# pacificclimate/VIC

Measured on AMD Instinct MI355X. Metric: cell-timesteps/s, higher is better.
Workload: dtype f64

## Files before the change

vic_amd/build.py:

```python
import os
import subprocess
import sys

HERE = os.path.dirname(os.path.abspath(__file__))
ROOT = os.path.dirname(HERE)
SRC = os.path.join(HERE, "csrc", "vicgpu_api.hip")
OUT = os.path.join(HERE, "libvicgpu.so")
HIPCC = os.environ.get("HIPCC", "/opt/rocm/bin/hipcc")
FLAGS = ["--offload-arch=gfx950", "-O3", "-ffp-contract=off", "-std=c++17", "-fPIC", "-shared", "-ftrivial-auto-var-init=zero",
         "-mllvm", "-sgpr-regalloc=basic",
         "-I" + os.path.join(ROOT, "include"), "-I" + os.path.join(HERE, "csrc")]


def needs_build():
    if not os.path.exists(OUT):
        return True
    t = os.path.getmtime(OUT)
    deps = [os.path.join(HERE, "csrc", f) for f in os.listdir(os.path.join(HERE, "csrc"))] + [os.path.join(ROOT, "include", f) for f in os.listdir(os.path.join(ROOT, "include"))]
    return any(os.path.getmtime(d) > t for d in deps)


RESOURCE_LIMITS = {
    "vic_hru_step<3, false>": (256, 3200),
    "vic_hru_step<3, true>": (256, 1800),
    "vic_hru_step<10, true>": (256, 2200),
    "vic_fd_stage<10, true, false>": (256, 800),
    "vic_fd_stage<10, false, false>": (256, 600),
    "vic_hru_step<50, true>": (256, 5200),
    "vic_fd_stage<50, true, false>": (256, 4500),
    "vic_fd_stage<50, true, true>": (256, 4500),
    "vic_fd_stage<50, false, false>": (256, 5300),
    "vic_fd_stage<50, false, true>": (256, 6300),
    "vic_surf_eval": (256, 0),
    "vic::vic_profile_solve_reg<10": (256, 128),
    "vic::vic_profile_solve_lockstep": (256, 0),
    "vic::vic_put_": (256, 0),
    "vic_cell_reduce": (128, 0),
}


def parse_resources(remarks):
    import re
    kern, cur = {}, None
    for line in remarks.splitlines():
        m = re.search(r"remark: .*?Function Name: (\S+)", line)
        if m:
            cur = m.group(1); kern[cur] = {}; continue
        m = re.search(r"remark: .*?\s{2,}([A-Za-z ]+?)(?: \[[^\]]*\])?: (\S+) \[-Rpass", line)
        if m and cur:
            kern[cur][m.group(1).strip()] = m.group(2)
    return kern


def resource_table(kern):
    import re
    names = list(kern)
    dem = subprocess.run(["c++filt"] + names, stdout=subprocess.PIPE, text=True).stdout.splitlines() if names else []
    rows = []
    for name, dm in zip(names, dem):
        v = kern[name]
        short = re.sub(r"\(.*", "", dm).replace("void ", "")
        rows.append((short, v.get("VGPRs", "?"), v.get("AGPRs", "?"), v.get("TotalSGPRs", "?"), v.get("ScratchSize", "?"),
                     v.get("VGPRs Spill", "?"), v.get("SGPRs Spill", "?"), v.get("Occupancy", "?")))
    rows.sort()
    return rows


def check_resources(rows):
    bad = []
    for r in rows:
        for prefix, (max_vgpr, max_scratch) in RESOURCE_LIMITS.items():
            if r[0].startswith(prefix):
                try:
                    if int(r[1]) > max_vgpr or int(r[4]) > max_scratch:
                        bad.append("%s: %s VGPRs, %s B scratch (limit %d / %d)" % (r[0], r[1], r[4], max_vgpr, max_scratch))
                except ValueError:
                    pass
    return bad


def build(force=False, extra=(), verbose=False, out=OUT):
    if not force and out == OUT and not needs_build():
        return OUT
    cmd = [HIPCC] + FLAGS + list(extra) + ["-Rpass-analysis=kernel-resource-usage", SRC, "-o", out]
    if verbose:
        print(" ".join(cmd))
    p = subprocess.run(cmd, stdout=subprocess.PIPE, stderr=subprocess.STDOUT, text=True)
    if p.returncode != 0:
        sys.stderr.write(p.stdout)
        raise subprocess.CalledProcessError(p.returncode, cmd)
    rows = resource_table(parse_resources(p.stdout))
    with open(os.path.splitext(out)[0] + ".resources.txt", "w") as f:
        f.write("%-62s %5s %5s %5s %8s %6s %6s %5s\n" % ("kernel", "VGPR", "AGPR", "SGPR", "scratchB", "vspill", "sspill", "occ"))
        for r in rows:
            f.write("%-62s %5s %5s %5s %8s %6s %6s %5s\n" % ((r[0][:62],) + r[1:]))
    bad = check_resources(rows)
    if bad and not extra:
        raise RuntimeError("kernel resource limits exceeded (vic_amd/build.py RESOURCE_LIMITS):\n  " + "\n  ".join(bad))
    return OUT


if __name__ == "__main__":
    args = [a for a in sys.argv[1:] if a != "-f"]
    out = OUT
    if "-o" in args:
        i = args.index("-o")
        out = os.path.abspath(args[i + 1])
        del args[i:i + 2]
    build(force="-f" in sys.argv, extra=args, verbose=True, out=out)
```

vic_amd/csrc/vicgpu_api.hip:

```cpp
#include <hip/hip_runtime.h>
#include <stdio.h>
#include <stdlib.h>
#include <string.h>
#include <algorithm>
#include <atomic>
#include <chrono>
#include <string>
#include <thread>
#include <vector>
#include "vicgpu.h"
#include <cstddef>
#include <type_traits>
#include "vic_glacier.hpp"
#include "vic_profile.hpp"
#include "vic_putdata.hpp"

using namespace vic;

#define HIPIGN(call) do { hipError_t ign_ = (call); (void)ign_; } while (0)
#define HIPCHK(ctx, call)                                                                              \
  do {                                                                                                 \
    hipError_t e_ = (call);                                                                            \
    if (e_ != hipSuccess) {                                                                            \
      (ctx)->err = std::string(#call) + ": " + hipGetErrorString(e_);                                  \
// ... 179 lines not shown
template <int NN>
VIC_DEV void load_state(const KArgs& a, int g, HruWork<NN>& w, bool node_props = true) {
  const int Nn = a.o.Nnode;
  const size_t nh = a.nhru;
  const double* __restrict__ sd = a.sd;
  const int* __restrict__ si = a.si;
#define SD(row) sd[(size_t)(row) * nh + g]
#define SI(row) si[(size_t)(row) * nh + g]
#pragma unroll
  for (int l = 0; l < 3; l++) { w.moist[l] = SD(SD_MOIST0 + l); w.ice[l] = SD(SD_ICE0 + l); w.layer_T[l] = SD(SD_LAYER_T0 + l); w.evap[l] = 0; }
  SoilEnergy& so = w.so; SnowEnergy& se = w.se; Snow& s = w.snow;
  so.snow_flux = SD(SD_SNOW_FLUX); so.grnd_flux = SD(SD_GRND_FLUX); so.deltaH = SD(SD_DELTAH); so.fusion = SD(SD_FUSION);
  so.LongUnderOut = SD(SD_LONGUNDEROUT); se.Tfoliage = SD(SD_TFOLIAGE);
  s.albedo = SD(SD_SNOW_ALBEDO); s.coldcontent = SD(SD_SNOW_COLDCONTENT); s.coverage = SD(SD_SNOW_COVERAGE);
  s.density = SD(SD_SNOW_DENSITY); s.depth = SD(SD_SNOW_DEPTH); s.pack_temp = SD(SD_SNOW_PACK_TEMP);
  s.pack_water = SD(SD_SNOW_PACK_WATER); s.snow_canopy = SD(SD_SNOW_CANOPY); s.surf_temp = SD(SD_SNOW_SURF_TEMP);
  s.surf_water = SD(SD_SNOW_SURF_WATER); s.swq = SD(SD_SNOW_SWQ); s.tmp_int_storage = SD(SD_SNOW_TMP_INT_STORAGE);
  s.store_swq = SD(SD_SNOW_STORE_SWQ); s.store_coverage = SD(SD_SNOW_STORE_COVERAGE); s.swq_slope = SD(SD_SNOW_SWQ_SLOPE);
  s.max_swq = SD(SD_SNOW_MAX_SWQ);
  s.blowing_flux = 0; s.canopy_vapor_flux = 0; s.mass_error = 0; s.melt = 0; s.Qnet = 0; s.surface_flux = 0; s.vapor_flux = 0;
  w.vv.Wdew = SD(SD_WDEW); w.vv.canopyevap = 0; w.vv.throughfall = 0;
  w.Tcanopy = SD(SD_TCANOPY); so.Tsurf = SD(SD_TSURF); se.AlbedoOver = SD(SD_ALBEDO_OVER); so.AlbedoUnder = SD(SD_ALBEDO_UNDER);
  se.canopy_advection = SD(SD_CANOPY_ADVECTION); se.canopy_latent = SD(SD_CANOPY_LATENT);
  se.canopy_latent_sub = SD(SD_CANOPY_LATENT_SUB); se.canopy_sensible = SD(SD_CANOPY_SENSIBLE);
  se.canopy_refreeze = SD(SD_CANOPY_REFREEZE);
  se.advected_sensible = so.advected_sensible = SD(SD_ADVECTED_SENSIBLE);
  se.advection = so.advection = SD(SD_ADVECTION);
  se.deltaCC = so.deltaCC = SD(SD_DELTACC);
  se.refreeze_energy = so.refreeze_energy = SD(SD_REFREEZE_ENERGY);
  so.melt_energy = SD(SD_MELT_ENERGY);
  se.error = so.error = SD(SD_ERROR);
  se.latent = so.latent = SD(SD_LATENT); se.latent_sub = so.latent_sub = SD(SD_LATENT_SUB);
  se.sensible = so.sensible = SD(SD_SENSIBLE);
  se.snow_flux = so.snow_flux;
  se.LongOverIn = SD(SD_LONGOVERIN); se.NetLongOver = SD(SD_NETLONGOVER); se.NetShortOver = SD(SD_NETSHORTOVER);
  se.ShortOverIn = SD(SD_SHORTOVERIN);
  so.NetShortGrnd = 0; so.NetLongUnder = SD(SD_NETLONGUNDER); so.NetShortUnder = 0;
  w.gl.surf_temp = SD(SD_GLAC_SURF_TEMP); w.gl.water_storage = SD(SD_GLAC_WATER_STORAGE);
  w.gl.cum_mass_balance = SD(SD_GLAC_CUM_MASS_BALANCE);
  w.gl.cold_content = NAN; w.gl.Qnet = NAN; w.gl.mass_balance = NAN; w.gl.ice_mass_balance = 0; w.gl.accumulation = NAN;
  w.gl.melt = NAN; w.gl.vapor_flux = NAN; w.gl.outflow = NAN; w.gl.outflow_coef = NAN; w.gl.inflow = NAN;
  w.deltaCC_glac = 0; w.glacier_flux = 0; w.glacier_melt_energy = 0;
  so.kappa[0] = so.kappa[1] = so.Cs[0] = so.Cs[1] = 0;
#pragma unroll
  for (int f = 0; f < 3; f++) { so.fdepth[f] = 0; so.tdepth[f] = 0; }
#pragma unroll
  for (int n = 0; n < NN; n++) {
    if (n < Nn) {
      w.nd.T[n] = SD(VICGPU_SD_NODE(SDN_T, n, Nn));
      if (node_props) {
        w.nd.moist[n] = SD(VICGPU_SD_NODE(SDN_MOIST, n, Nn)); w.nd.ice[n] = SD(VICGPU_SD_NODE(SDN_ICE, n, Nn));
        w.nd.kappa[n] = SD(VICGPU_SD_NODE(SDN_KAPPA, n, Nn)); w.nd.Cs[n] = SD(VICGPU_SD_NODE(SDN_CS, n, Nn));
      } else { w.nd.moist[n] = 0; w.nd.ice[n] = 0; w.nd.kappa[n] = 0; w.nd.Cs[n] = 0; }
      w.nd.fbflag[n] = SI(VICGPU_SI_NODE(SIN_T_FBFLAG, n, Nn)); w.nd.fbcount[n] = SI(VICGPU_SI_NODE(SIN_T_FBCOUNT, n, Nn));
    } else {
      w.nd.T[n] = 0; w.nd.moist[n] = 0; w.nd.ice[n] = 0; w.nd.kappa[n] = 0; w.nd.Cs[n] = 0; w.nd.fbflag[n] = 0; w.nd.fbcount[n] = 0;
    }
  }
  s.last_snow = SI(SI_SNOW_LAST_SNOW); s.MELTING = SI(SI_SNOW_MELTING); s.snow = SI(SI_SNOW_SNOW); s.store_snow = SI(SI_SNOW_STORE_SNOW);
  s.surf_temp_fbcount = SI(SI_SNOW_SURF_TEMP_FBCOUNT); s.surf_temp_fbflag = SI(SI_SNOW_SURF_TEMP_FBFLAG);
  so.Tsurf_fbcount = SI(SI_TSURF_FBCOUNT); so.Tsurf_fbflag = SI(SI_TSURF_FBFLAG);
  se.Tfoliage_fbcount = SI(SI_TFOLIAGE_FBCOUNT); se.Tfoliage_fbflag = SI(SI_TFOLIAGE_FBFLAG);
  so.frozen = SI(SI_FROZEN); so.Nfrost = SI(SI_NFROST); so.Nthaw = SI(SI_NTHAW);
  w.gl.surf_temp_fbcount = SI(SI_GLAC_SURF_TEMP_FBCOUNT); w.gl.surf_temp_fbflag = SI(SI_GLAC_SURF_TEMP_FBFLAG);
#undef SD
#undef SI
}

template <int NN>
VIC_DEV void load_node_props(const KArgs& a, int g, Nodes<NN>& nd) {
  const int Nn = a.o.Nnode;
  const size_t nh = a.nhru;
  const double* __restrict__ sd = a.sd;
#pragma unroll
  for (int n = 0; n < NN; n++) {
    if (n < Nn) {
      nd.moist[n] = sd[(size_t)VICGPU_SD_NODE(SDN_MOIST, n, Nn) * nh + g]; nd.ice[n] = sd[(size_t)VICGPU_SD_NODE(SDN_ICE, n, Nn) * nh + g];
      nd.kappa[n] = sd[(size_t)VICGPU_SD_NODE(SDN_KAPPA, n, Nn) * nh + g]; nd.Cs[n] = sd[(size_t)VICGPU_SD_NODE(SDN_CS, n, Nn) * nh + g];
    }
  }
}

template <int NN>
VIC_DEV void load_untouched_state(const KArgs& a, int g, HruWork<NN>& w) {
  const int Nn = a.o.Nnode;
  const size_t nh = a.nhru;
  const double* __restrict__ sd = a.sd;
  const int* __restrict__ si = a.si;
#pragma unroll
  for (int l = 0; l < 3; l++) {
    w.moist[l] = sd[(size_t)(SD_MOIST0 + l) * nh + g]; w.ice[l] = sd[(size_t)(SD_ICE0 + l) * nh + g];
    w.layer_T[l] = sd[(size_t)(SD_LAYER_T0 + l) * nh + g]; w.evap[l] = 0;
  }
  w.vv.Wdew = sd[(size_t)SD_WDEW * nh + g]; w.vv.canopyevap = 0; w.vv.throughfall = 0;
  SoilEnergy& so = w.so;
  so.deltaCC = 0; so.refreeze_energy = 0; so.deltaH = 0; so.fusion = 0; so.grnd_flux = 0; so.latent = 0; so.latent_sub = 0; so.sensible = 0;
  so.snow_flux = 0; so.error = 0; so.NetShortGrnd = 0; so.NetLongUnder = 0; so.NetShortUnder = 0; so.LongUnderOut = 0; so.AlbedoUnder = 0;
  so.melt_energy = 0; so.Tsurf = 0; so.kappa[0] = so.kappa[1] = so.Cs[0] = so.Cs[1] = 0;
#pragma unroll
  for (int f = 0; f < 3; f++) { so.fdepth[f] = 0; so.tdepth[f] = 0; }
  so.advected_sensible = sd[(size_t)SD_ADVECTED_SENSIBLE * nh + g];
  so.Tsurf_fbflag = 0; so.Tsurf_fbcount = si[(size_t)SI_TSURF_FBCOUNT * nh + g];
  so.frozen = 0; so.Nfrost = 0; so.Nthaw = si[(size_t)SI_NTHAW * nh + g];
  w.Tcanopy = 0;
  w.gl.surf_temp = sd[(size_t)SD_GLAC_SURF_TEMP * nh + g]; w.gl.water_storage = sd[(size_t)SD_GLAC_WATER_STORAGE * nh + g];
  w.gl.cum_mass_balance = sd[(size_t)SD_GLAC_CUM_MASS_BALANCE * nh + g];
  w.gl.cold_content = NAN; w.gl.Qnet = NAN; w.gl.mass_balance = NAN; w.gl.ice_mass_balance = 0; w.gl.accumulation = NAN;
  w.gl.melt = NAN; w.gl.vapor_flux = NAN; w.gl.outflow = NAN; w.gl.outflow_coef = NAN; w.gl.inflow = NAN;
  w.gl.surf_temp_fbcount = si[(size_t)SI_GLAC_SURF_TEMP_FBCOUNT * nh + g]; w.gl.surf_temp_fbflag = si[(size_t)SI_GLAC_SURF_TEMP_FBFLAG * nh + g];
  w.deltaCC_glac = 0; w.glacier_flux = 0; w.glacier_melt_energy = 0;
#pragma unroll
  for (int n = 0; n < NN; n++) {
    w.nd.T[n] = 0; w.nd.moist[n] = 0; w.nd.ice[n] = 0; w.nd.kappa[n] = 0; w.nd.Cs[n] = 0; w.nd.fbflag[n] = 0;
    w.nd.fbcount[n] = (n < Nn) ? si[(size_t)VICGPU_SI_NODE(SIN_T_FBCOUNT, n, Nn) * nh + g] : 0;
  }
#pragma unroll
  for (int p = 0; p < NPET; p++) w.pot_evap[p] = 0;
}

template <int NN>
VIC_DEV void store_state(const KArgs& a, int g, const HruWork<NN>& w) {
  const int Nn = a.o.Nnode;
  const size_t nh = a.nhru;
  double* __restrict__ sd = a.sd;
  int* __restrict__ si = a.si;
#define SD(row) sd[(size_t)(row) * nh + g]
#define SI(row) si[(size_t)(row) * nh + g]
#pragma unroll
  for (int l = 0; l < 3; l++) { SD(SD_MOIST0 + l) = w.moist[l]; SD(SD_ICE0 + l) = w.ice[l]; SD(SD_LAYER_T0 + l) = w.layer_T[l]; }
  const SoilEnergy& so = w.so; const SnowEnergy& se = w.se; const Snow& s = w.snow;
  SD(SD_SNOW_FLUX) = so.snow_flux; SD(SD_GRND_FLUX) = so.grnd_flux; SD(SD_DELTAH) = so.deltaH; SD(SD_FUSION) = so.fusion;
  SD(SD_LONGUNDEROUT) = so.LongUnderOut; SD(SD_TFOLIAGE) = se.Tfoliage;
  SD(SD_SNOW_ALBEDO) = s.albedo; SD(SD_SNOW_COLDCONTENT) = s.coldcontent; SD(SD_SNOW_COVERAGE) = s.coverage;
  SD(SD_SNOW_DENSITY) = s.density; SD(SD_SNOW_DEPTH) = s.depth; SD(SD_SNOW_PACK_TEMP) = s.pack_temp;
  SD(SD_SNOW_PACK_WATER) = s.pack_water; SD(SD_SNOW_CANOPY) = s.snow_canopy; SD(SD_SNOW_SURF_TEMP) = s.surf_temp;
  SD(SD_SNOW_SURF_WATER) = s.surf_water; SD(SD_SNOW_SWQ) = s.swq; SD(SD_SNOW_TMP_INT_STORAGE) = s.tmp_int_storage;
  SD(SD_SNOW_STORE_SWQ) = s.store_swq; SD(SD_SNOW_STORE_COVERAGE) = s.store_coverage; SD(SD_SNOW_SWQ_SLOPE) = s.swq_slope;
  SD(SD_SNOW_MAX_SWQ) = s.max_swq; SD(SD_WDEW) = w.vv.Wdew;
  SD(SD_TCANOPY) = w.Tcanopy; SD(SD_TSURF) = so.Tsurf; SD(SD_ALBEDO_OVER) = w.AlbedoOver_avg; SD(SD_ALBEDO_UNDER) = so.AlbedoUnder;
  SD(SD_CANOPY_ADVECTION) = se.canopy_advection; SD(SD_CANOPY_LATENT) = se.canopy_latent;
  SD(SD_CANOPY_LATENT_SUB) = se.canopy_latent_sub; SD(SD_CANOPY_SENSIBLE) = se.canopy_sensible;
  SD(SD_CANOPY_REFREEZE) = se.canopy_refreeze; SD(SD_ADVECTED_SENSIBLE) = so.advected_sensible;
  SD(SD_ADVECTION) = so.advection; SD(SD_DELTACC) = so.deltaCC; SD(SD_REFREEZE_ENERGY) = so.refreeze_energy;
  SD(SD_MELT_ENERGY) = so.melt_energy; SD(SD_ERROR) = so.error; SD(SD_LATENT) = so.latent; SD(SD_LATENT_SUB) = so.latent_sub;
  SD(SD_SENSIBLE) = so.sensible; SD(SD_LONGOVERIN) = w.LongOverIn_avg; SD(SD_NETLONGOVER) = w.NetLongOver_avg;
  SD(SD_NETSHORTOVER) = w.NetShortOver_avg; SD(SD_SHORTOVERIN) = w.ShortOverIn_avg; SD(SD_NETLONGUNDER) = so.NetLongUnder;
  SD(SD_GLAC_SURF_TEMP) = w.gl.surf_temp; SD(SD_GLAC_WATER_STORAGE) = w.gl.water_storage;
  SD(SD_GLAC_CUM_MASS_BALANCE) = w.gl.cum_mass_balance;
#pragma unroll
  for (int n = 0; n < NN; n++) {
    if (n < Nn) {
      SD(VICGPU_SD_NODE(SDN_T, n, Nn)) = w.nd.T[n]; SD(VICGPU_SD_NODE(SDN_MOIST, n, Nn)) = w.nd.moist[n];
      SD(VICGPU_SD_NODE(SDN_ICE, n, Nn)) = w.nd.ice[n]; SD(VICGPU_SD_NODE(SDN_KAPPA, n, Nn)) = w.nd.kappa[n];
      SD(VICGPU_SD_NODE(SDN_CS, n, Nn)) = w.nd.Cs[n];
      SI(VICGPU_SI_NODE(SIN_T_FBFLAG, n, Nn)) = w.nd.fbflag[n]; SI(VICGPU_SI_NODE(SIN_T_FBCOUNT, n, Nn)) = w.nd.fbcount[n];
    }
  }
  SI(SI_SNOW_LAST_SNOW) = s.last_snow; SI(SI_SNOW_MELTING) = s.MELTING; SI(SI_SNOW_SNOW) = s.snow; SI(SI_SNOW_STORE_SNOW) = s.store_snow;
  SI(SI_SNOW_SURF_TEMP_FBCOUNT) = s.surf_temp_fbcount; SI(SI_SNOW_SURF_TEMP_FBFLAG) = s.surf_temp_fbflag;
  SI(SI_TSURF_FBCOUNT) = so.Tsurf_fbcount; SI(SI_TSURF_FBFLAG) = so.Tsurf_fbflag;
  SI(SI_TFOLIAGE_FBCOUNT) = se.Tfoliage_fbcount; SI(SI_TFOLIAGE_FBFLAG) = se.Tfoliage_fbflag;
  SI(SI_FROZEN) = so.frozen; SI(SI_NFROST) = so.Nfrost; SI(SI_NTHAW) = so.Nthaw;
  SI(SI_GLAC_SURF_TEMP_FBCOUNT) = w.gl.surf_temp_fbcount; SI(SI_GLAC_SURF_TEMP_FBFLAG) = w.gl.surf_temp_fbflag;
#undef SD
#undef SI
}
// ... 144 lines not shown
#pragma unroll
  for (int p = 0; p < NPET; p++) C.aero_pet[p] = ap[p];
  C.Ra = Ra; C.U = U; C.disp = disp; C.zref = zref; C.z0 = z0;
  C.overstory = overstory ? 1 : 0;
  w.aero_resist_surface = Ra.v[SNOW_FREE];
  w.aero_resist_overstory = Ra.v[CANOPY];
#pragma unroll
  for (int p = 0; p < NPET; p++) w.pot_evap[p] = 0;
  return err;
}

template <int NN>
VIC_DEV void hru_epilogue(const KArgs& a, int g, const CellView& cv, const Soil3& s3, const StepConst& C, HruWork<NN>& w, int err, bool glac) {
  w.rootmoist = 0; w.wetness = 0;
#pragma unroll
  for (int l = 0; l < 3; l++) {
    if (C.root[l] > 0) w.rootmoist += w.moist[l];
    w.wetness += (w.moist[l] - s3.Wpwp[l]) / (cv.lay(CPL_POROSITY, l) * s3.depth[l] * 1000 - s3.Wpwp[l]);
  }
  w.wetness /= 3;

  bool finite = true;
#pragma unroll
  for (int l = 0; l < 3; l++) finite = finite && isfinite(w.moist[l]);
  finite = finite && isfinite(w.nd.T[0]) && isfinite(w.snow.swq);
  if (!finite) err |= VICGPU_CELLERR_NAN;

  PROF_T0(t_store);
  store_state<NN>(a, g, w);
  store_flux<NN>(a, g, w, glac);
  a.hru_err[g] = err;
  PROF_ADD(8, t_store);
}

template <int NN, bool GLAC>
__global__ __launch_bounds__(64) void vic_hru_step(const KArgs a) {
  const int gi = a.map.index(blockIdx.x, threadIdx.x, a.gcount);
  if (gi < 0) return;
  const int g = a.glist ? a.glist[gi] : gi;
  const Opt& o = a.o;
  const HruId id = hru_id(a, g);
  if (id.is_glacier != GLAC && id.run) return;
  if (!id.run) {
    if (!GLAC) store_zero_record(a, g);
    return;
  }
  PROF_T0(t_kernel);
  CellView cv{a.cell_params, a.ncell, id.c, o.Nnode, o.Nband};
  VegLib vl{a.veglib};
  Forcing fc{a.forcing, a.snowflag, a.ncell, id.c, o.NR + 1};
  const Soil3 s3 = load_soil3(cv);
  HruWork<NN> w;
  StepConst C;
  int err = hru_prologue<NN, GLAC>(a, g, id, cv, vl, fc, s3, w, C);
  PROF_ADD(1, t_kernel);

  if (!(err & VICGPU_CELLERR_AERO)) {
    bool ok;
    if constexpr (GLAC) {
      GlacEnergy ge;
      double nlu, nsu, sui;
      const double blow[4] = {C.sigma_slope, C.lag_one, C.fetch, (double)C.is_art_bare};
      ok = surface_fluxes_glac<NN>(o, cv, vl, s3, fc, a.dmy, C.veg_idx, C.band, C.bare_albedo, C.aero_pet, C.Ra, C.U, C.zref, C.z0, C.disp, blow, w, w.gl,
                                   w.so.NetLongUnder, ge, nlu, nsu, sui);
      SoilEnergy& so = w.so; SnowEnergy& se = w.se;
      so.snow_flux = ge.snow_flux; so.grnd_flux = ge.grnd_flux; so.deltaH = 0; so.fusion = 0; so.LongUnderOut = ge.LongUnderOut;
      so.AlbedoUnder = ge.AlbedoUnder; so.advected_sensible = ge.advected_sensible; so.advection = ge.advection;
      so.deltaCC = ge.deltaCC; so.refreeze_energy = ge.refreeze_energy; so.error = ge.error; so.latent = ge.latent;
      so.latent_sub = ge.latent_sub; so.sensible = ge.sensible; so.NetLongUnder = nlu; so.NetShortUnder = nsu; so.NetShortGrnd = 0;
      se.canopy_advection = 0; se.canopy_latent = 0; se.canopy_latent_sub = 0; se.canopy_sensible = 0; se.canopy_refreeze = 0;
      w.AlbedoOver_avg = 0; w.LongOverIn_avg = 0; w.NetLongOver_avg = 0; w.NetShortOver_avg = 0; w.ShortOverIn_avg = 0;
      w.ShortUnderIn_avg = sui;
      w.deltaCC_glac = ge.deltaCC_glac; w.glacier_flux = ge.glacier_flux; w.glacier_melt_energy = ge.glacier_melt_energy;
      if (!isnan(w.gl.cum_mass_balance) && !isnan(w.gl.mass_balance)) w.gl.cum_mass_balance += w.gl.mass_balance;
    } else {
      ok = surface_fluxes<NN>(o, cv, vl, s3, fc, a.dmy, C, w);
    }
    if (!ok) err |= VICGPU_CELLERR_SOLVER;
  }
  hru_epilogue<NN>(a, g, cv, s3, C, w, err, GLAC);
  PROF_ADD(0, t_kernel);
  PROF_WAVE(0);
  PROF_LANE(1);
}

template <int NN, bool FIRST, bool MULTI>
__global__ __launch_bounds__(64) VIC_WAVES_PER_EU(1, 1) void vic_fd_stage(const KArgs a) {
  const int gi = a.map.index(blockIdx.x, threadIdx.x, a.gcount);
  if (gi < 0) return;
  const int g = a.glist ? a.glist[gi] : gi;
  const Opt& o = a.o;
  const HruId id = hru_id(a, g);
  if (id.run && id.is_glacier) return;
  if (FIRST && !id.run) { store_zero_record(a, g); a.hstate[g] = 0; return; }
  if (!FIRST && (a.hstate[g] & HS_STATE) != 2) return;
  CellView cv{a.cell_params, a.ncell, id.c, o.Nnode, o.Nband};
  VegLib vl{a.veglib};
  Forcing fc{a.forcing, a.snowflag, a.ncell, id.c, o.NR + 1};
  const Soil3 s3 = load_soil3(cv);
  const int Nn = node_count<NN>(o.Nnode);
  const CtxRef cx = CtxRef::at(a.ctx, ctx_words<NN>(), g);
  HruWork<NN> w;
  StepConst C;
  SubLoop L;
  int err = 0;
  bool more;
  PROF_T0(t_stage);
  if constexpr (FIRST) {
    err = hru_prologue<NN, false>(a, g, id, cv, vl, fc, s3, w, C, false);
    PROF_ADD(1, t_stage);
    more = !(err & VICGPU_CELLERR_AERO);
    if (more) sf_begin<NN>(o, fc, C, w, L);
  } else {
    SubStep P;
    SurfEB eb;
    SurfSolve sv;
    ctx_get_words(cx, CO_SV, sv, (int)CW_SV_ITER, (int)CW_SV);
    ctx_get(cx, CO_EBM, static_cast<SurfEBMut&>(eb));
    ctx_get_words(cx, CO_EBC, static_cast<SurfEBConst&>(eb), 0, EBC_W_POST);
    surf_cell_fill(eb, cv, vl, s3, fc, eb.hidx, id.veg_idx, a.dmy.month);
    ctx_get(cx, CO_P, P);
    ctx_get_words(cx, CO_L, L, 0, (int)CW_L_HEAD);
    if (MULTI && L.N_steps > 0) ctx_get_words(cx, CO_L, L, (int)CW_L_HEAD, (int)CW_L);
    else zero_substep_sums(L);
    load_untouched_state<NN>(a, g, w);
    if constexpr (MULTI) {
      ctx_get(cx, CO_C, C);
      WCarryMulti<NN> km;
      ctx_get(cx, CO_WM, km);
      carry_in_multi<NN>(km, w);
    } else {
      StepConstPost q;
      ctx_get(cx, CO_C, q);
      step_const_post_in(q, P.UnderStory, C);
      C.veg_idx = id.veg_idx; C.band = id.band; C.is_art_bare = id.is_art_bare ? 1 : 0;
      C.overstory = (vl.f(id.veg_idx, VL_OVERSTORY) != 0.0) ? 1 : 0;
#pragma unroll
      for (int l = 0; l < 3; l++) C.root[l] = (double)(float)a.hpd[(size_t)(HPD_ROOT0 + l) * a.nhru + g];
    }
    {
      WCarry k;
      ctx_get(cx, CO_W, k);
      carry_in<NN>(k, w);
    }
    PROF_ADD(11, t_stage);
    PROF_T0(t_post);
    const double* __restrict__ po = a.pout + (size_t)g * pout_hru_stride(Nn) + sv.final_slot * pout_stride(Nn);
    const int* __restrict__ poc = reinterpret_cast<const int*>(po + Nn + 1);
    double Tprof[NN];
    int cntprof[NN];
    const unsigned long long flags = (unsigned long long)__double_as_longlong(po[Nn]);
#pragma unroll
    for (int n = 0; n < NN; n++) {
      Tprof[n] = (n < Nn) ? po[n] : 0.0;
      cntprof[n] = (n < Nn) ? poc[n] : 0;
    }
    using mask_t = typename NodeBound<NN>::mask_t;
    sf_sub_post<NN>(o, cv, vl, s3, fc, a.dmy, C, w, L, P, eb, sv, Tprof, cntprof,
                    (mask_t)(flags & ((1ull << NodeBound<NN>::ok_bit) - 1ull)));
    PROF_ADD(12, t_post);
    more = true;
  }
  bool pend = false;
  int key = 0;
  if ((FIRST || MULTI) && more && L.hidx < L.endhidx) {
    if constexpr (FIRST || MULTI) {
      SubStep P;
      SurfEB eb;
      SurfSolve sv;
      PROF_T0(t_pre);
      sf_sub_pre<NN>(o, cv, vl, s3, fc, a.dmy, C, w, L, P, eb, sv);
      PROF_ADD(13, t_pre);
      PROF_T0(t_put);
      ctx_put(cx, CO_SV, sv);
      ctx_put_words(cx, CO_EBM, static_cast<const SurfEBMut&>(eb), 0, EBM_W_KEEP);
      const int cls = surf_eb_class(eb);
      ebc_put(cx, eb, cls);
      ctx_put(cx, CO_P, P);
      ctx_put_words(cx, CO_L, L, 0, (int)CW_L_HEAD);
      if (MULTI && L.N_steps > 0) ctx_put_words(cx, CO_L, L, (int)CW_L_HEAD, (int)CW_L);
      if constexpr (MULTI) {
        if (FIRST) ctx_put(cx, CO_C, C);
        WCarryMulti<NN> km;
        carry_out_multi<NN>(w, km);
        ctx_put(cx, CO_WM, km);
      } else {
        StepConstPost q;
        step_const_post_out(C, P.UnderStory, q);
        ctx_put(cx, CO_C, q);
      }
      {
        WCarry k;
        carry_out<NN>(w, k);
        ctx_put(cx, CO_W, k);
      }
      load_node_props<NN>(a, g, w.nd);
      {
        int nfrozen = 0;
        bool kink = false;
#pragma unroll
        for (int n = 1; n < NN; n++)
          if (n < Nn && eb.frozen_on) {
            if (w.nd.T[n] < 0) nfrozen++;
            if (fabs(w.nd.T[n]) < SOIL_DT) kink = true;
          }
        if constexpr (NN >= NBUCKET / 2) nfrozen = (nfrozen < NBUCKET / 2 - 1) ? nfrozen : NBUCKET / 2 - 1;
        key = nfrozen + (kink ? NBUCKET / 2 : 0);
        a.hkey[g] = key;
      }
      profile_item_store<NN>(o, cv, s3, w.nd, eb.delta_t, eb.frozen_on != 0, a.pin + (size_t)g * Nn * PREC);
      if (o.IMPLICIT) {
        double* __restrict__ im = a.pimp + (size_t)g * Nn * PIMP;
#pragma unroll
        for (int n = 0; n < NN; n++)
          if (n < Nn) {
            im[n * PIMP + PI_MOIST] = w.nd.moist[n]; im[n * PIMP + PI_ICE] = (n == 0) ? eb.delta_t : w.nd.ice[n];
            im[n * PIMP + PI_KAPPA] = w.nd.kappa[n]; im[n * PIMP + PI_CS] = w.nd.Cs[n];
          }
        a.lastexp[g] = -1;
      }
      a.ts[g] = sv.x;
      a.pslot[g] = 0;
      if (o.QUICK_SOLVE) {
        int tmpNnodes = 0;
#pragma unroll
        for (int n = NN - 1; n >= 0; n--)
          if (n <= Nn - 5 && w.nd.T[n] >= 0 && w.nd.T[(n + 1 < NN) ? n + 1 : n] < 0) tmpNnodes = n + 1;
        if (tmpNnodes == 0) tmpNnodes = (w.nd.T[0] <= 0 && w.nd.T[1] >= 0) ? Nn : 3;
        else tmpNnodes += 4;
        a.jl[g] = (sv.stage == SurfSolve::ROOT_QUICK) ? tmpNnodes - 1 : (o.NOFLUX ? Nn : Nn - 1);
      }
      a.pout[(size_t)g * pout_hru_stride(Nn) + pout_key(Nn, 0)] = NAN;
      a.pout[(size_t)g * pout_hru_stride(Nn) + pout_key(Nn, 1)] = NAN;
      a.hstate[g] = 1 | (cls << HS_CLS_SHIFT);
      pend = true;
      PROF_ADD(14, t_put);
    }
  } else {
    PROF_T0(t_end);
    if (more && !sf_end<NN>(o, cv, s3, C, w, L)) err |= VICGPU_CELLERR_SOLVER;
    PROF_ADD(15, t_end);
    hru_epilogue<NN>(a, g, cv, s3, C, w, err, false);
    a.hstate[g] = 0;
  }
  list_append(a.list, a.count, a.list_cap, pend, key, g);
  PROF_ADD(0, t_stage);
  PROF_WAVE(0);
  PROF_LANE(1);
}

struct EArgs {
  Opt o;
  LaunchMap map;
  int ncell, nhru, Nn;
  const int* glist;
  int gcount;
  const double* cell_params;
  const int* hpi;
  unsigned long long* ctx;
  size_t ctx_words;
  double* pout;
  int* pslot;
  double* ts;
  int* jl;
  int* hstate;
  int* list_next;
  int* count_next;
  int list_cap;
  const int* hkey;
  int* profile_next;
  int* evalonly;
  int* eo_list_next;
  int list_thr;
  const int* list_cur;
  const int* count_cur;
  const int* eo_list_cur;
  const int* npend_cur;
  int implicit;
  const double* veglib;
  const double* forcing;
  int month;
};

constexpr int EVAL_WAVES = 2;
__global__ __launch_bounds__(64) VIC_WAVES_PER_EU(EVAL_WAVES, EVAL_WAVES) void vic_surf_eval(const EArgs a) {
  if (blockIdx.x == 0 && threadIdx.x == 0) *a.profile_next = 0;
  const int npend = *a.npend_cur;
  int g;
  if (npend <= a.list_thr) {
    if ((int)blockIdx.x * 64 >= npend) return;
    __shared__ int bcount[NBUCKET];
    for (int b = threadIdx.x; b < NBUCKET; b += 64) bcount[b] = a.count_cur[b];
    __syncthreads();
    int nsolve = 0;
#pragma unroll 1
    for (int b = 0; b < NBUCKET; b++) nsolve += bcount[b];
    const int gi = blockIdx.x * 64 + threadIdx.x;
    if (gi >= npend) return;
    if (gi < nsolve) {
      int rem = gi, found = 0;
#pragma unroll 1
      for (int b = 0; b < NBUCKET; b++) {
// ... 424 lines not shown
  bool domain_ready = false;
  double *d_veglib = nullptr, *d_cp = nullptr, *d_hpd = nullptr, *d_sd = nullptr, *d_flux = nullptr, *d_forcing = nullptr,
         *d_cell_out = nullptr, *d_accum = nullptr;
  int *d_hpi = nullptr, *d_si = nullptr, *d_cell_off = nullptr, *d_cell_list = nullptr, *d_hru_err = nullptr, *d_cell_err = nullptr;
  unsigned char* d_snowflag = nullptr;
  std::vector<int> dmy;
  int chunk_steps = 0;
  struct ForcingSlot {
    double *d_f = nullptr, *d_raw = nullptr;
    unsigned char* d_s = nullptr;
    size_t fcap = 0, scap = 0, rawcap = 0, stage_cap = 0;
    void* h_stage = nullptr;
    std::vector<int> dmy;
    int nsteps = 0;
    hipEvent_t uploaded = nullptr;
    hipEvent_t released = nullptr;
    bool upload_pending = false, was_current = false;
  } slot[2];
  int cur = -1, staged = -1;
  hipStream_t stream = nullptr, copy_stream = nullptr;
  bool own_stream = true;
  std::vector<hipEvent_t> ev;
  int ev_used = 0;
  int write_fluxes = 1;
  int steps_done = 0;
  bool any_glacier = false;
  bool fd = false;
  unsigned long long* d_ctx = nullptr;
  double *d_pin = nullptr, *d_ts = nullptr, *d_pout = nullptr;
  int *d_hstate = nullptr, *d_pslot = nullptr, *d_hkey = nullptr, *d_lastexp = nullptr, *d_jl = nullptr;
  double* d_pimp = nullptr;
  int profile_waves = 0;
  int eval_list_pct = 30;
  bool node_newton = false;
  std::vector<FdChunk> chunks;
  int ev_steps = 0;
  bool put_on = false;
  int out_step_ratio = 1, out_nrow = 0;
  OutLayout out_lay;
  double *d_out_data = nullptr, *d_out_agg = nullptr, *d_pb = nullptr;
  unsigned char* d_rowagg = nullptr;
};

static void free_domain(vicgpu_ctx* c) {
  void* ps[] = {c->d_cp, c->d_hpd, c->d_sd, c->d_flux, c->d_cell_out, c->d_accum, c->d_hpi, c->d_si, c->d_cell_off, c->d_cell_list,
                c->d_hru_err, c->d_cell_err, c->d_ctx, c->d_pin, c->d_ts, c->d_pout, c->d_hstate, c->d_pslot, c->d_hkey,
                c->d_out_data, c->d_out_agg, c->d_pb, c->d_rowagg, c->d_pimp, c->d_lastexp, c->d_jl};
  for (void* p : ps) HIPIGN(hipFree(p));
  c->d_out_data = c->d_out_agg = c->d_pb = nullptr;
  c->d_rowagg = nullptr;
  c->d_pimp = nullptr; c->d_lastexp = nullptr; c->d_jl = nullptr;
  c->put_on = false;
  for (FdChunk& ch : c->chunks) {
    HIPIGN(hipFree(ch.d_glist)); HIPIGN(hipFree(ch.d_list[0])); HIPIGN(hipFree(ch.d_list[1])); HIPIGN(hipFree(ch.d_count));
    HIPIGN(hipFree(ch.d_elist[0])); HIPIGN(hipFree(ch.d_elist[1]));
    HIPIGN(hipFree(ch.d_fb_list)); HIPIGN(hipFree(ch.d_fb_count));
    if (ch.h_count) HIPIGN(hipHostFree(ch.h_count));
    if (ch.done) HIPIGN(hipEventDestroy(ch.done));
    for (hipEvent_t e : ch.readback) if (e) HIPIGN(hipEventDestroy(e));
    if (ch.stream) HIPIGN(hipStreamDestroy(ch.stream));
  }
  c->chunks.clear();
  c->domain_ready = false;
  c->chunk_steps = 0;
  c->dmy.clear();
  c->cur = c->staged = -1;
  c->d_forcing = nullptr; c->d_snowflag = nullptr;
  c->d_ctx = nullptr; c->d_pin = c->d_ts = c->d_pout = nullptr; c->d_hstate = c->d_pslot = c->d_hkey = nullptr;
  c->d_cp = c->d_hpd = c->d_sd = c->d_flux = c->d_cell_out = c->d_accum = nullptr;
  c->d_hpi = c->d_si = c->d_cell_off = c->d_cell_list = c->d_hru_err = c->d_cell_err = nullptr;
}

template <int NN>
static hipError_t launch_hru(const KArgs& ka, hipStream_t st, bool ordinary, bool glacier) {
  const int nblk = ka.map.nblocks(ka.gcount);
  if constexpr (NN == 3) {
    if (ordinary) hipLaunchKernelGGL((vic_hru_step<NN, false>), dim3(nblk), dim3(64), 0, st, ka);
  }
  if (glacier) hipLaunchKernelGGL((vic_hru_step<NN, true>), dim3(nblk), dim3(64), 0, st, ka);
  return hipGetLastError();
}

template <int NN>
static hipError_t launch_fd_stage(const KArgs& ka, bool multi, hipStream_t st) {
  const dim3 grid(ka.map.nblocks(ka.gcount)), block(64);
  if (ka.phase == 0) {
    if (multi) hipLaunchKernelGGL((vic_fd_stage<NN, true, true>), grid, block, 0, st, ka);
    else hipLaunchKernelGGL((vic_fd_stage<NN, true, false>), grid, block, 0, st, ka);
  } else {
    if (multi) hipLaunchKernelGGL((vic_fd_stage<NN, false, true>), grid, block, 0, st, ka);
    else hipLaunchKernelGGL((vic_fd_stage<NN, false, false>), grid, block, 0, st, ka);
  }
  return hipGetLastError();
}

template <int NN>
static hipError_t launch_profile(const PArgs& pa, int nmax, int resident_waves, bool newton, hipStream_t st) {
  int nblk = (nmax + 63) / 64;
  if (nblk > resident_waves) nblk = resident_waves;
  if (nblk < 1) nblk = 1;
  const dim3 g(nblk), b(64);
  if constexpr (NN == 10) {
    if (newton) hipLaunchKernelGGL((vic_profile_solve_reg<NN, true>), g, b, 0, st, pa);
    else hipLaunchKernelGGL((vic_profile_solve_reg<NN, false>), g, b, 0, st, pa);
  } else {
    if (newton) hipLaunchKernelGGL((vic_profile_solve_lockstep<NN, true>), g, b, 0, st, pa);
    else hipLaunchKernelGGL((vic_profile_solve_lockstep<NN, false>), g, b, 0, st, pa);
  }
  return hipGetLastError();
}

template <int NN>
static int profile_resident_waves(int device, bool newton) {
  int per_cu = 0, ncu = 0;
  hipError_t e;
  if constexpr (NN == 10) e = newton ? hipOccupancyMaxActiveBlocksPerMultiprocessor(&per_cu, vic_profile_solve_reg<NN, true>, 64, 0)
                                     : hipOccupancyMaxActiveBlocksPerMultiprocessor(&per_cu, vic_profile_solve_reg<NN, false>, 64, 0);
  else e = newton ? hipOccupancyMaxActiveBlocksPerMultiprocessor(&per_cu, vic_profile_solve_lockstep<NN, true>, 64, 0)
                  : hipOccupancyMaxActiveBlocksPerMultiprocessor(&per_cu, vic_profile_solve_lockstep<NN, false>, 64, 0);
  if (e != hipSuccess || per_cu <= 0) per_cu = 8;
  if (hipDeviceGetAttribute(&ncu, hipDeviceAttributeMultiprocessorCount, device) != hipSuccess || ncu <= 0) ncu = 256;
  return per_cu * ncu;
}

#define CHKCH(ch, call)                                                                               \
  do {                                                                                                 \
    hipError_t e_ = (call);                                                                            \
    if (e_ != hipSuccess) {                                                                            \
      (ch)->err = std::string(#call) + ": " + hipGetErrorString(e_);                                   \
      return VICGPU_ERR_HIP;                                                                           \
    }                                                                                                  \
  } while (0)

constexpr int CNT_LIST_STRIDE = 64, CNT_CURSOR = 128, CNT_EVALONLY = 160, CNT_EVALONLY_STRIDE = 32, CNT_NPEND = 224, CNT_TOTAL = 256;
static_assert(NBUCKET <= CNT_LIST_STRIDE, "counter block layout");
static inline int* cnt_list(int* d_count, int l) { return d_count + l * CNT_LIST_STRIDE; }
static inline int* cnt_evalonly(int* d_count, int l) { return d_count + CNT_EVALONLY + l * CNT_EVALONLY_STRIDE; }

static int fd_read_count(FdChunk* ch, int which, int* nsolve, int* nevalonly) {
  CHKCH(ch, hipMemcpyAsync(ch->h_count, ch->d_count, sizeof(int) * CNT_TOTAL, hipMemcpyDeviceToHost, ch->stream));
  CHKCH(ch, hipStreamSynchronize(ch->stream));
  int n = 0;
  for (int b = 0; b < NBUCKET; b++) n += ch->h_count[which * CNT_LIST_STRIDE + b];
  *nsolve = n;
  *nevalonly = ch->h_count[CNT_EVALONLY + which * CNT_EVALONLY_STRIDE];
  return VICGPU_OK;
}

#define NODE_DISPATCH(Nnode, F, ...)                                                                                          \
  (node_bound(Nnode) == 10 ? F<10>(__VA_ARGS__)                                                                           \
                           : node_bound(Nnode) == VIC_MID_NODES ? F<VIC_MID_NODES>(__VA_ARGS__) : F<VIC_MAX_NODES>(__VA_ARGS__))

static int fd_step(vicgpu_ctx* c, FdChunk* ch, KArgs ka) {
  const int Nn = c->o.Nnode;
  hipStream_t st = ch->stream;
  if (c->any_glacier) CHKCH(ch, NODE_DISPATCH(Nn, launch_hru, ka, st, false, true));
  CHKCH(ch, hipMemsetAsync(ch->d_count, 0, sizeof(int) * CNT_TOTAL, st));
  int cur = 0;
  ka.phase = 0; ka.list = ch->d_list[cur]; ka.count = cnt_list(ch->d_count, cur); ka.list_cap = ch->list_cap;
  CHKCH(ch, NODE_DISPATCH(Nn, launch_fd_stage, ka, c->o.NF > 1, st));
  PArgs pa;
  pa.pin = c->d_pin; pa.ts = c->d_ts; pa.pout = c->d_pout; pa.pslot = c->d_pslot; pa.Nn = Nn; pa.NOFLUX = c->o.NOFLUX; pa.EXP_TRANS = c->o.EXP_TRANS;
  pa.TFALLBACK = c->o.TFALLBACK; pa.next = ch->d_count + CNT_CURSOR; pa.cap = ch->list_cap; pa.jl = c->d_jl;
  EArgs ea;
  ea.o = c->o; ea.ncell = c->ncell; ea.nhru = c->nhru; ea.Nn = Nn; ea.glist = ch->d_glist; ea.gcount = ch->gcount; ea.map = ch->map;
  ea.cell_params = c->d_cp; ea.hpi = c->d_hpi; ea.ctx = c->d_ctx;
  ea.ctx_words = NODE_DISPATCH(Nn, ctx_words);
  ea.pout = c->d_pout; ea.pslot = c->d_pslot; ea.ts = c->d_ts; ea.hstate = c->d_hstate; ea.profile_next = ch->d_count + CNT_CURSOR;
  ea.list_thr = (int)((long long)ch->gcount * c->eval_list_pct / 100);
  ea.list_cap = ch->list_cap; ea.hkey = c->d_hkey; ea.implicit = c->o.IMPLICIT; ea.jl = c->d_jl;
  ea.veglib = c->d_veglib; ea.forcing = ka.forcing; ea.month = ka.dmy.month;
  const bool trace_rounds = getenv("VICGPU_TRACE_ROUNDS") != nullptr;
  const int FREE_ROUNDS = 6;
  const int nsub = c->o.NF;
  for (int p = 1; p <= nsub; p++) {
    int nmax = ch->gcount;
    int npend = -1;
    int rb_list[RB_DEPTH];
    int rb_first = -1;
    for (int round = 0;; round++) {
      pa.list = ch->d_list[cur]; pa.count = cnt_list(ch->d_count, cur); pa.count_zero = cnt_list(ch->d_count, cur ^ 1);
      pa.evalonly_zero = cnt_evalonly(ch->d_count, cur ^ 1);
      pa.pend_counts = cnt_list(ch->d_count, cur); pa.pend_eo = cnt_evalonly(ch->d_count, cur); pa.pend_out = ch->d_count + CNT_NPEND;
      if (c->o.IMPLICIT) {
        CHKCH(ch, hipMemsetAsync(ch->d_fb_count, 0, sizeof(int) * (NBUCKET + 1), st));
        IArgs ia;
        ia.ncell = c->ncell; ia.nhru = c->nhru; ia.Nband = c->o.Nband; ia.pimp = c->d_pimp; ia.hpi = c->d_hpi; ia.cell_params = c->d_cp;
        ia.hkey = c->d_hkey; ia.fb_list = ch->d_fb_list; ia.fb_count = ch->d_fb_count; ia.lastexp = c->d_lastexp; ia.cursor = ch->d_fb_count + NBUCKET;
        {
          int nblk = (nmax + 63) / 64;
          if (nblk > 4096) nblk = 4096;
          if (nblk < 1) nblk = 1;
          hipLaunchKernelGGL(vic_profile_solve_implicit, dim3(nblk), dim3(64), 0, st, pa, ia);
        }
        CHKCH(ch, hipGetLastError());
        pa.list = ch->d_fb_list; pa.count = ch->d_fb_count;
      }
      CHKCH(ch, NODE_DISPATCH(Nn, launch_profile, pa, nmax, c->profile_waves, c->node_newton, st));
      ea.list_next = ch->d_list[cur ^ 1]; ea.count_next = cnt_list(ch->d_count, cur ^ 1);
      ea.evalonly = cnt_evalonly(ch->d_count, cur ^ 1); ea.eo_list_next = ch->d_elist[cur ^ 1];
      ea.list_cur = ch->d_list[cur]; ea.count_cur = cnt_list(ch->d_count, cur);
      ea.eo_list_cur = ch->d_elist[cur]; ea.npend_cur = ch->d_count + CNT_NPEND;
      const bool sparse = npend >= 0 && npend <= ea.list_thr;
      hipLaunchKernelGGL(vic_surf_eval, dim3(sparse ? ((npend + 63) / 64 > 0 ? (npend + 63) / 64 : 1) : ea.map.nblocks(ch->gcount)), dim3(64), 0, st, ea);
      CHKCH(ch, hipGetLastError());
      cur ^= 1;
      ch->rounds++;
      if (trace_rounds) {
        int n = 0, ne = 0;
        if (fd_read_count(ch, cur, &n, &ne) != VICGPU_OK) return VICGPU_ERR_HIP;
        fprintf(stderr, "vicgpu rounds: chunk %d sub-step %d round %d leaves %d solves + %d evaluation-only of %d\n", (int)(ch - &c->chunks[0]), p, round, n, ne, ch->gcount);
      }
      if (round + 2 >= FREE_ROUNDS) {
        const int slot = round % RB_DEPTH;
        if (rb_first < 0) rb_first = round;
        CHKCH(ch, hipMemcpyAsync(ch->h_count + slot * CNT_TOTAL, ch->d_count, sizeof(int) * CNT_TOTAL, hipMemcpyDeviceToHost, st));
        CHKCH(ch, hipEventRecord(ch->readback[slot], st));
        rb_list[slot] = cur;
      }
      if (rb_first >= 0 && round - RB_LAG >= rb_first) {
        const int slot = (round - RB_LAG) % RB_DEPTH;
        CHKCH(ch, hipEventSynchronize(ch->readback[slot]));
        const int* h = ch->h_count + slot * CNT_TOTAL;
        int n = 0;
        for (int b = 0; b < NBUCKET; b++) n += h[rb_list[slot] * CNT_LIST_STRIDE + b];
        const int neo = h[CNT_EVALONLY + rb_list[slot] * CNT_EVALONLY_STRIDE];
        if (n == 0 && neo == 0) break;
        nmax = n;
        npend = n + neo;
      }
    }
    ka.phase = p; ka.list = ch->d_list[cur]; ka.count = cnt_list(ch->d_count, cur);
    CHKCH(ch, NODE_DISPATCH(Nn, launch_fd_stage, ka, c->o.NF > 1, st));
    if (p < nsub) {
      int n = 0, ne = 0;
      const int r = fd_read_count(ch, cur, &n, &ne);
      if (r != VICGPU_OK) return r;
      if (n == 0) break;
    }
  }
  ch->steps++;
  return VICGPU_OK;
// ... 961 lines not shown
```

Measured before the change: 3.853 million.

## Split profile item setup out of fd stage into separate kernel for NF==1

For the single-subcycle case, the per-HRU profile input setup (freeze-bucket key, profile item store, implicit-solver state) moves out of the large fd_stage kernel into a new lightweight vic_profile_items kernel launched just before it. The fd stage then reads the precomputed key from hkey instead of loading node properties and writing the profile buffers itself. This is meant to lower register pressure and code size in the heavy fd_stage kernel. The cost is an extra launch and a second pass that re-reads soil parameters and node state from global memory.

After: 3.774 million. 0.98x the previous value.

```diff
diff --git a/vic_amd/build.py b/vic_amd/build.py
--- a/vic_amd/build.py
+++ b/vic_amd/build.py
@@ -31,6 +31,7 @@
     "vic_fd_stage<50, true, true>": (256, 4500),
     "vic_fd_stage<50, false, false>": (256, 5300),
     "vic_fd_stage<50, false, true>": (256, 6300),
+    "vic_profile_items<10>": (160, 0),
     "vic_surf_eval": (256, 0),
     "vic::vic_profile_solve_reg<10": (256, 128),
     "vic::vic_profile_solve_lockstep": (256, 0),
diff --git a/vic_amd/csrc/vicgpu_api.hip b/vic_amd/csrc/vicgpu_api.hip
--- a/vic_amd/csrc/vicgpu_api.hip
+++ b/vic_amd/csrc/vicgpu_api.hip
@@ -285,6 +285,38 @@
 }
 
 template <int NN>
+VIC_DEV int profile_items_put(const KArgs& a, int g, const CellView& cv, const Soil3& s3, const Nodes<NN>& nd, double delta_t, int frozen_on) {
+  const Opt& o = a.o;
+  const int Nn = node_count<NN>(o.Nnode);
+  int key;
+  {
+    int nfrozen = 0;
+    bool kink = false;
+#pragma unroll
+    for (int n = 1; n < NN; n++)
+      if (n < Nn && frozen_on) {
+        if (nd.T[n] < 0) nfrozen++;
+        if (fabs(nd.T[n]) < SOIL_DT) kink = true;
+      }
+    if constexpr (NN >= NBUCKET / 2) nfrozen = (nfrozen < NBUCKET / 2 - 1) ? nfrozen : NBUCKET / 2 - 1;
+    key = nfrozen + (kink ? NBUCKET / 2 : 0);
+    a.hkey[g] = key;
+  }
+  profile_item_store<NN>(o, cv, s3, nd, delta_t, frozen_on != 0, a.pin + (size_t)g * Nn * PREC);
+  if (o.IMPLICIT) {
+    double* __restrict__ im = a.pimp + (size_t)g * Nn * PIMP;
+#pragma unroll
+    for (int n = 0; n < NN; n++)
+      if (n < Nn) {
+        im[n * PIMP + PI_MOIST] = nd.moist[n]; im[n * PIMP + PI_ICE] = (n == 0) ? delta_t : nd.ice[n];
+        im[n * PIMP + PI_KAPPA] = nd.kappa[n]; im[n * PIMP + PI_CS] = nd.Cs[n];
+      }
+    a.lastexp[g] = -1;
+  }
+  return key;
+}
+
+template <int NN>
 VIC_DEV void load_untouched_state(const KArgs& a, int g, HruWork<NN>& w) {
   const int Nn = a.o.Nnode;
   const size_t nh = a.nhru;
@@ -595,6 +627,25 @@
   PROF_ADD(0, t_kernel);
   PROF_WAVE(0);
   PROF_LANE(1);
+}
+
+template <int NN>
+__global__ __launch_bounds__(64) void vic_profile_items(const KArgs a) {
+  const int gi = a.map.index(blockIdx.x, threadIdx.x, a.gcount);
+  if (gi < 0) return;
+  const int g = a.glist ? a.glist[gi] : gi;
+  const Opt& o = a.o;
+  const HruId id = hru_id(a, g);
+  if (!id.run || id.is_glacier) return;
+  CellView cv{a.cell_params, a.ncell, id.c, o.Nnode, o.Nband};
+  const Soil3 s3 = load_soil3(cv);
+  const int Nn = o.Nnode;
+  Nodes<NN> nd;
+#pragma unroll
+  for (int n = 0; n < NN; n++) nd.T[n] = (n < Nn) ? a.sd[(size_t)VICGPU_SD_NODE(SDN_T, n, Nn) * a.nhru + g] : 0.0;
+  load_node_props<NN>(a, g, nd);
+  const int frozen_on = (cv.s(CP_FS_ACTIVE) != 0.0) && o.FROZEN_SOIL;
+  profile_items_put<NN>(a, g, cv, s3, nd, (double)o.dt * 3600., frozen_on);
 }
 
 template <int NN, bool FIRST, bool MULTI>
@@ -707,30 +758,11 @@
         carry_out<NN>(w, k);
         ctx_put(cx, CO_W, k);
       }
-      load_node_props<NN>(a, g, w.nd);
-      {
-        int nfrozen = 0;
-        bool kink = false;
-#pragma unroll
-        for (int n = 1; n < NN; n++)
-          if (n < Nn && eb.frozen_on) {
-            if (w.nd.T[n] < 0) nfrozen++;
-            if (fabs(w.nd.T[n]) < SOIL_DT) kink = true;
-          }
-        if constexpr (NN >= NBUCKET / 2) nfrozen = (nfrozen < NBUCKET / 2 - 1) ? nfrozen : NBUCKET / 2 - 1;
-        key = nfrozen + (kink ? NBUCKET / 2 : 0);
-        a.hkey[g] = key;
-      }
-      profile_item_store<NN>(o, cv, s3, w.nd, eb.delta_t, eb.frozen_on != 0, a.pin + (size_t)g * Nn * PREC);
-      if (o.IMPLICIT) {
-        double* __restrict__ im = a.pimp + (size_t)g * Nn * PIMP;
-#pragma unroll
-        for (int n = 0; n < NN; n++)
-          if (n < Nn) {
-            im[n * PIMP + PI_MOIST] = w.nd.moist[n]; im[n * PIMP + PI_ICE] = (n == 0) ? eb.delta_t : w.nd.ice[n];
-            im[n * PIMP + PI_KAPPA] = w.nd.kappa[n]; im[n * PIMP + PI_CS] = w.nd.Cs[n];
-          }
-        a.lastexp[g] = -1;
+      if constexpr (MULTI) {
+        load_node_props<NN>(a, g, w.nd);
+        key = profile_items_put<NN>(a, g, cv, s3, w.nd, eb.delta_t, eb.frozen_on);
+      } else {
+        key = a.hkey[g];
       }
       a.ts[g] = sv.x;
       a.pslot[g] = 0;
@@ -1321,6 +1353,12 @@
 }
 
 template <int NN>
+static hipError_t launch_profile_items(const KArgs& ka, hipStream_t st) {
+  hipLaunchKernelGGL((vic_profile_items<NN>), dim3(ka.map.nblocks(ka.gcount)), dim3(64), 0, st, ka);
+  return hipGetLastError();
+}
+
+template <int NN>
 static hipError_t launch_fd_stage(const KArgs& ka, bool multi, hipStream_t st) {
   const dim3 grid(ka.map.nblocks(ka.gcount)), block(64);
   if (ka.phase == 0) {
@@ -1397,6 +1435,7 @@
   CHKCH(ch, hipMemsetAsync(ch->d_count, 0, sizeof(int) * CNT_TOTAL, st));
   int cur = 0;
   ka.phase = 0; ka.list = ch->d_list[cur]; ka.count = cnt_list(ch->d_count, cur); ka.list_cap = ch->list_cap;
+  if (c->o.NF == 1) CHKCH(ch, NODE_DISPATCH(Nn, launch_profile_items, ka, st));
   CHKCH(ch, NODE_DISPATCH(Nn, launch_fd_stage, ka, c->o.NF > 1, st));
   PArgs pa;
   pa.pin = c->d_pin; pa.ts = c->d_ts; pa.pout = c->d_pout; pa.pslot = c->d_pslot; pa.Nn = Nn; pa.NOFLUX = c->o.NOFLUX; pa.EXP_TRANS = c->o.EXP_TRANS;
```
